# siravan/fib_tf

Hardware: AMD Instinct MI355X
Metric: million cell-steps/sec (grid_cells x timesteps / wall_s), 4v 512x512 (higher is better)
Workload: dtype f32; 1 GPU; fenton 512x512, dt=0.1 ms, phase-field hole, S1 + S2 pacing (BASELINE configs[1]); 1 step = 1 run() tick = 10 sub-steps; sub_steps_per_tick=10, fused_sub_steps_per_launch=10, launches_per_tick=1, ticks_per_launch=32, tile=44x25 cells, 3 rows per wave (chosen by measurement on the first tick), arithmetic=fast_math (default policy), parallelism=single device, setup_ticks=6001, timing=one region of 2647 ticks

## Files before the change

fib_tf_amd/_lib.py:

```python
import ctypes as C
import os
import subprocess

import numpy as np

HERE = os.path.dirname(os.path.abspath(__file__))
ROOT = os.path.dirname(HERE)
SO = os.path.join(HERE, 'libfibhip.so')
SRC = os.path.join(HERE, 'csrc', 'fibhip.hip')
HDR = os.path.join(ROOT, 'include', 'fibhip.h')

FENTON4V, BR, COURT, COURT_US, CUSTOM = 0, 1, 2, 3, 4
OBS_MAPS = ('first_up', 'last_up', 'prev_up', 'apd', 'count')
CHEBY, SKIP, CHRONIC, FAST, ALLVARS, ROW_INTERLEAVED, ZEROPAD, HOLD = 1, 2, 4, 8, 16, 32, 64, 128

HIPCC_FLAGS = ['-O3', '--offload-arch=gfx950', '-ffp-contract=off', '-fno-slp-vectorize', '-fvisibility=hidden', '-fPIC', '-shared',
               '-std=c++17', '-Wall', '-Wno-unused-value', '-Wno-unused-result']


def _build_tag(so_path):
    import re
    return '-DFIB_BUILD_TAG=b_' + re.sub(r'[^0-9A-Za-z_]', '_', os.path.splitext(os.path.basename(so_path))[0])


# ... 102 lines not shown
    'fibhip_comm_open': ([C.c_char_p], C.c_int),
    'fibhip_comm_unique_id': ([C.c_char_p], C.c_int),
    'fibhip_comm_check': ([_h, C.c_int, C.c_int], C.c_int),
    'fibhip_comm_init': ([_h, C.c_char_p, C.c_int, C.c_int], C.c_int),
    'fibhip_comm_exchange': ([_h, C.c_int, C.c_int], C.c_int),
    'fibhip_comm_free': ([_h], C.c_int),
    'fibhip_copy_bandwidth': ([C.c_int, C.c_size_t, C.c_int, _fp], C.c_int),
    'fibhip_warm': ([C.c_int], C.c_int),
    'fibhip_module_load': ([C.c_int, C.c_void_p, C.c_size_t, C.POINTER(ModuleDesc), C.POINTER(C.c_void_p)], C.c_int),
    'fibhip_module_unload': ([C.c_void_p], C.c_int),
    'fibhip_launch_plan': ([_h, _ip, _ip], C.c_int),
    'fibhip_get_state_direct': ([_h, C.c_int, _fp], C.c_int),
    'fibhip_host_alloc': ([C.c_size_t, C.POINTER(C.c_void_p)], C.c_int),
    'fibhip_host_free': ([C.c_void_p], C.c_int),
    'fibhip_ticks_per_launch': ([_h], C.c_int),
    'fibhip_launch_stats': ([_h, C.POINTER(C.c_longlong)], C.c_int),
    'fibhip_spec_stats': ([_h, C.POINTER(C.c_longlong)], C.c_int),
    'fibhip_fallbacks': ([_h, C.POINTER(C.c_longlong)], C.c_int),
    'fibhip_set_mt_wait_ms': ([_h, C.c_int], C.c_int),
    'fibhip_expect': ([_h, C.c_int], C.c_int),
    'fibhip_trace_begin': ([_h], C.c_int),
    'fibhip_trace_end': ([_h, C.POINTER(TraceEvent), C.c_int], C.c_int),
    'fibhip_plan_tile': ([_h, _ip, _ip, _ip], C.c_int),
    'fibhip_observe_begin': ([_h, C.c_int, C.c_float, C.c_float], C.c_int),
    'fibhip_observe_get': ([_h, C.c_int, C.c_void_p], C.c_int),
    'fibhip_observe_ticks': ([_h, C.POINTER(C.c_longlong)], C.c_int),
    'fibhip_observe_end': ([_h], C.c_int),
    'fibhip_electrode_begin': ([_h, C.c_int, C.c_int, _ip, _fp, C.c_int, C.c_longlong], C.c_int),
    'fibhip_electrode_count': ([_h, C.POINTER(C.c_longlong)], C.c_int),
    'fibhip_electrode_read': ([_h, C.c_longlong, C.c_longlong, _fp], C.c_int),
    'fibhip_electrode_end': ([_h], C.c_int),
    'fibhip_last_error': ([], C.c_char_p),
}

_lib = None


DEPS = [SRC, HDR] + [os.path.join(HERE, "csrc", f) for f in ("kernels.hpp", "models.hpp", "fenton_step.inc", "br_step.inc",
                                                             "court_step.inc", "court_inter.inc")]


def build(force=False, verbose=False):
    if not force and os.path.exists(SO) and all(os.path.getmtime(SO) >= os.path.getmtime(d) for d in DEPS):
        return SO
    hipcc = os.environ.get('HIPCC', '/opt/rocm/bin/hipcc')
    cmd = [hipcc] + HIPCC_FLAGS + [SRC, '-o', SO]
# ... 474 lines not shown
```

fib_tf_amd/csrc/fibhip.hip:

```cpp
#include <hip/hip_runtime.h>

#include <atomic>
#include <chrono>
#include <climits>
#include <cmath>
#include <cstdarg>
#include <cstdio>
#include <cstdlib>
#include <cstring>
#include <dlfcn.h>
#include <limits>
#include <mutex>
#include <new>
#include <vector>

#include "../../include/fibhip.h"
#include "kernels.hpp"

using namespace fib;

static thread_local char g_err[512] = "";

static int fail(int code, const char *fmt, ...)
{
// ... 61 lines not shown
}

template <class M, class P, int MODE, int K, int TX, int TY, int R, bool PHASE>
static hipError_t launch_strip(hipStream_t st, const LaunchCtx &c)
{
    Geo g = c.g;
    g.tiles_x = (g.W + TX - 1) / TX;
    g.ty_a = (g.r1 > g.r0) ? (g.r1 - g.r0 + TY - 1) / TY : 0;
    const int tiles_y = g.ty_a + ((g.rb1 > g.rb0) ? (g.rb1 - g.rb0 + TY - 1) / TY : 0);
    g.ntiles = g.tiles_x * tiles_y;
    if (g.ntiles <= 0) return hipSuccess;
    PtrTab<M::NVAR> pt;
    for (int v = 0; v < M::NVAR; ++v) {
        pt.in[v] = c.in[v];
        pt.out[v] = c.out[v];
    }
    constexpr int NT = 64 * ((TY + 2 * (K - 1) + R - 1) / R);
    const int grid = ((g.ntiles + 7) / 8) * 8;
    hipLaunchKernelGGL((strip_kernel<M, P, MODE, K, TX, TY, R, PHASE>), dim3(grid), dim3(NT), 0, st, g, pt, c.ph,
                       *static_cast<const typename M::Consts *>(c.consts), c.sub0);
    return hipGetLastError();
}

template <class M, class P, int MODE, int K, int TX, int TY, int R, bool PHASE>
static hipError_t launch_strip_mt(hipStream_t st, const LaunchCtx &c)
{
    Geo g = c.g;
    g.tiles_x = (g.W + TX - 1) / TX;
    g.ty_a = (g.r1 > g.r0) ? (g.r1 - g.r0 + TY - 1) / TY : 0;
    g.ntiles = g.tiles_x * g.ty_a;
    if (g.ntiles <= 0) return hipSuccess;
    PtrTab<M::NVAR> pt;
    for (int v = 0; v < M::NVAR; ++v) {
        pt.in[v] = c.in[v];
        pt.out[v] = c.out[v];
    }
    constexpr int NT = 64 * ((TY + 2 * (K - 1) + R - 1) / R);
    const int grid = ((g.ntiles + 7) / 8) * 8;
    hipLaunchKernelGGL((strip_mt_kernel<M, P, MODE, K, TX, TY, R, PHASE>), dim3(grid), dim3(NT), 0, st, g, pt, c.ph,
                       *static_cast<const typename M::Consts *>(c.consts), c.sub0, c.mt);
    return hipGetLastError();
}

template <class M, class P, int MODE, int K, int TX, int TY, int R, bool PHASE>
static hipError_t launch_rows(hipStream_t st, const LaunchCtx &c)
{
    Geo g = c.g;
    g.tiles_x = (g.W + TX - 1) / TX;
    g.ty_a = (g.r1 > g.r0) ? (g.r1 - g.r0 + TY - 1) / TY : 0;
    const int tiles_y = g.ty_a + ((g.rb1 > g.rb0) ? (g.rb1 - g.rb0 + TY - 1) / TY : 0);
    g.ntiles = g.tiles_x * tiles_y;
    if (g.ntiles <= 0) return hipSuccess;
    PtrTab<M::NVAR> pt;
    for (int v = 0; v < M::NVAR; ++v) {
        pt.in[v] = c.in[v];
        pt.out[v] = c.out[v];
    }
    constexpr int NT = 64 * ((TY + 2 * (K - 1) + R - 1) / R);
    const int grid = ((g.ntiles + 7) / 8) * 8;
    hipLaunchKernelGGL((rows_kernel<M, P, MODE, K, TX, TY, R, PHASE>), dim3(grid), dim3(NT), 0, st, g, pt, c.ph,
                       *static_cast<const typename M::Consts *>(c.consts), c.sub0);
    return hipGetLastError();
// ... 40 lines not shown
    auto put = [&](const void *p, size_t n, size_t align) {
        off = (off + align - 1) & ~(align - 1);
        memcpy(buf + off, p, n);
        off += n;
    };
    put(&g, sizeof g, alignof(Geo));
    off = (off + 7) & ~(size_t)7;
    memcpy(buf + off, c.in, (size_t)c.nvar * sizeof(void *));
    off += (size_t)c.nvar * sizeof(void *);
    memcpy(buf + off, c.out, (size_t)c.nvar * sizeof(void *));
    off += (size_t)c.nvar * sizeof(void *);
    if (c.kind != MK_POINTWISE) put(&c.ph, sizeof c.ph, alignof(PhaseTab));
    const char zeros[64] = {0};
    if (c.consts_bytes > 0) put(c.consts ? c.consts : zeros, (size_t)c.consts_bytes, 4);
    if (c.kind != MK_POINTWISE) put(&c.sub0, sizeof c.sub0, alignof(int));
    if (c.kind == MK_STRIP_MT) put(&c.mt, sizeof c.mt, alignof(MtArgs));
    void *config[] = {HIP_LAUNCH_PARAM_BUFFER_POINTER, buf, HIP_LAUNCH_PARAM_BUFFER_SIZE, &off, HIP_LAUNCH_PARAM_END};
    return hipModuleLaunchKernel(c.kern, grid, 1, 1, threads, 1, 1, 0, st, nullptr, config);
}

constexpr int VM_FENTON_ZP = 100;
constexpr int VM_COURT_AGG = 101;

struct Variant {
    int model, mode, fast, phase;
    int K, TX, TY, NT;
    launch_fn fn;
    hipFunction_t kern = nullptr;
    int kind = 0;
    launch_fn fn_mt = nullptr;
    hipFunction_t kern_mt = nullptr;
};

#define V4(MODEL, MID, MODE, K, TX, TY, NT)                                                        \
    {MID, MODE, 0, 0, K, TX, TY, NT, launch_tick<MODEL, Exact, MODE, K, TX, TY, NT, false>},       \
    {MID, MODE, 0, 1, K, TX, TY, NT, launch_tick<MODEL, Exact, MODE, K, TX, TY, NT, true>},        \
    {MID, MODE, 1, 0, K, TX, TY, NT, launch_tick<MODEL, Fast, MODE, K, TX, TY, NT, false>},        \
    {MID, MODE, 1, 1, K, TX, TY, NT, launch_tick<MODEL, Fast, MODE, K, TX, TY, NT, true>}

#define F2(MODEL, MID, MODE, K, TX, TY, NT)                                                        \
    {MID, MODE, 1, 0, K, TX, TY, NT, launch_tick<MODEL, Fast, MODE, K, TX, TY, NT, false>},        \
    {MID, MODE, 1, 1, K, TX, TY, NT, launch_tick<MODEL, Fast, MODE, K, TX, TY, NT, true>}

#define FS2(MODEL, MID, MODE, K, TX, TY, R)                                                        \
    {MID, MODE, 1, 0, K, TX, TY, -(R), launch_strip<MODEL, Fast, MODE, K, TX, TY, R, false>},      \
    {MID, MODE, 1, 1, K, TX, TY, -(R), launch_strip<MODEL, Fast, MODE, K, TX, TY, R, true>}

#define S4(MODEL, MID, MODE, K, TX, TY, R)                                                         \
    {MID, MODE, 0, 0, K, TX, TY, -(R), launch_strip<MODEL, Exact, MODE, K, TX, TY, R, false>},     \
    {MID, MODE, 0, 1, K, TX, TY, -(R), launch_strip<MODEL, Exact, MODE, K, TX, TY, R, true>},      \
    {MID, MODE, 1, 0, K, TX, TY, -(R), launch_strip<MODEL, Fast, MODE, K, TX, TY, R, false>},      \
    {MID, MODE, 1, 1, K, TX, TY, -(R), launch_strip<MODEL, Fast, MODE, K, TX, TY, R, true>}

#define S4M(MODEL, MID, MODE, K, TX, TY, R)                                                        \
    {MID, MODE, 0, 0, K, TX, TY, -(R), launch_strip<MODEL, Exact, MODE, K, TX, TY, R, false>, nullptr, 0,  \
     launch_strip_mt<MODEL, Exact, MODE, K, TX, TY, R, false>},                                    \
    {MID, MODE, 0, 1, K, TX, TY, -(R), launch_strip<MODEL, Exact, MODE, K, TX, TY, R, true>, nullptr, 0,   \
     launch_strip_mt<MODEL, Exact, MODE, K, TX, TY, R, true>},                                     \
    {MID, MODE, 1, 0, K, TX, TY, -(R), launch_strip<MODEL, Fast, MODE, K, TX, TY, R, false>, nullptr, 0,   \
     launch_strip_mt<MODEL, Fast, MODE, K, TX, TY, R, false>},                                     \
    {MID, MODE, 1, 1, K, TX, TY, -(R), launch_strip<MODEL, Fast, MODE, K, TX, TY, R, true>, nullptr, 0,    \
     launch_strip_mt<MODEL, Fast, MODE, K, TX, TY, R, true>}

#define W4(MODEL, MID, MODE, K, TX, TY, R)                                                         \
    {MID, MODE, 0, 0, K, TX, TY, -(32 + (R)), launch_rows<MODEL, Exact, MODE, K, TX, TY, R, false>},  \
    {MID, MODE, 0, 1, K, TX, TY, -(32 + (R)), launch_rows<MODEL, Exact, MODE, K, TX, TY, R, true>},   \
    {MID, MODE, 1, 0, K, TX, TY, -(32 + (R)), launch_rows<MODEL, Fast, MODE, K, TX, TY, R, false>},   \
    {MID, MODE, 1, 1, K, TX, TY, -(32 + (R)), launch_rows<MODEL, Fast, MODE, K, TX, TY, R, true>}

static const Variant g_variants[] = {
#ifdef FIB_CUSTOM_MODEL_INC
    V4(Custom, FIBHIP_CUSTOM, 0, 1, 64, 4, 256),
#if FIB_CUSTOM_K > 1
    S4(Custom, FIBHIP_CUSTOM, 0, FIB_CUSTOM_K, FIB_CUSTOM_TX, FIB_CUSTOM_TY, FIB_CUSTOM_R),
#if FIB_CUSTOM_TYB > 0
    S4(Custom, FIBHIP_CUSTOM, 0, FIB_CUSTOM_K, FIB_CUSTOM_TX, FIB_CUSTOM_TYB, FIB_CUSTOM_R),
#endif
#endif
#if FIB_CUSTOM_K2 > 1 && FIB_CUSTOM_K2 != FIB_CUSTOM_K
    S4(Custom, FIBHIP_CUSTOM, 0, FIB_CUSTOM_K2, FIB_CUSTOM_TX2, FIB_CUSTOM_TY2, FIB_CUSTOM_R2),
#endif
#endif
#ifndef FIB_CUSTOM_ONLY
#ifndef FIB_ONLY_BR
    S4M(Fenton, FIBHIP_FENTON4V, 0, 10, 44, 25, 3),
    S4M(Fenton, FIBHIP_FENTON4V, 0, 10, 44, 28, 3),
    S4M(Fenton, FIBHIP_FENTON4V, 0, 10, 44, 27, 3),
    S4M(Fenton, FIBHIP_FENTON4V, 0, 10, 44, 30, 3),
    S4M(Fenton, FIBHIP_FENTON4V, 0, 10, 44, 32, 4),
    S4M(Fenton, FIBHIP_FENTON4V, 0, 10, 44, 36, 4),
    S4M(Fenton, FIBHIP_FENTON4V, 0, 10, 44, 40, 4),
    S4M(Fenton, FIBHIP_FENTON4V, 0, 10, 44, 44, 4),
    S4(Fenton, FIBHIP_FENTON4V, 0, 5, 54, 21, 3),
    S4(Fenton, FIBHIP_FENTON4V, 0, 5, 54, 23, 3),
    S4(Fenton, FIBHIP_FENTON4V, 0, 5, 54, 22, 4),
    S4(Fenton, FIBHIP_FENTON4V, 0, 5, 54, 27, 3),
    S4(Fenton, FIBHIP_FENTON4V, 0, 5, 54, 25, 3),
    S4(Fenton, FIBHIP_FENTON4V, 0, 5, 54, 28, 3),
    S4(Fenton, FIBHIP_FENTON4V, 0, 5, 54, 31, 3),
    S4(Fenton, FIBHIP_FENTON4V, 0, 5, 54, 34, 3),
    S4(Fenton, FIBHIP_FENTON4V, 0, 5, 54, 32, 4),
    S4(Fenton, FIBHIP_FENTON4V, 0, 5, 54, 40, 3),
    S4(Fenton, FIBHIP_FENTON4V, 0, 5, 54, 44, 4),
    S4(Fenton, FIBHIP_FENTON4V, 0, 5, 54, 56, 4),
    S4(Fenton, FIBHIP_FENTON4V, 0, 2, 60, 18, 4),
    W4(Fenton, FIBHIP_FENTON4V, 0, 10, 44, 25, 3),
    W4(Fenton, FIBHIP_FENTON4V, 0, 5, 54, 21, 3),
    V4(Fenton, FIBHIP_FENTON4V, 0, 10, 32, 32, 512),
// ... 107 lines not shown
    int cur[FIB_MAXVAR];
    int nxt[FIB_MAXVAR];
    bool has_consts;
    Fenton::Consts kf;
    BeelerReuter::Consts kb;
    Courtemanche::Consts kc;
#ifdef FIB_CUSTOM_MODEL_INC
    Custom::Consts ku;
#endif
    std::vector<PlanItem> plan;
    hipEvent_t ev_main, ev_int, ev_t0, ev_t1;
    int phase_of_tick;
    long launches, t_launches0;
    int own0, own1;
    bool whole_in_edges;
    int pending;
    int multi_max;
    std::vector<PlanItem> plan_multi[4];
    float *xbuf;
    unsigned *epochs;
    unsigned epoch_base;
    bool epochs_stale;
    int mt_max;
    int mt_cur;
    long long n_ticks, n_mt_launches, n_mt_ticks;
    long long n_spec_kept, n_spec_redone;
    int mt_run, mt_run_prev;
    int spec_n, spec_used;
    int spec_nxt[FIB_MAXVAR];
    int mt_run_prev2;
    int hist[8], nhist;
    bool series_fresh;
    bool ahead_ok;
    unsigned spec_id;
    unsigned *host_word;
    unsigned *done_word, *done_word_dev;
    unsigned done_seq;
    bool no_stream_write;
    unsigned *snap_flags_dev;
    unsigned mt_ids;
    unsigned mt_seq;
    bool spec_trust;
    hipEvent_t ev_spec;
    unsigned *snap_flags;
    unsigned snap_seq;
    bool mt_inflight;
// ... 423 lines not shown
        const char *e = getenv("FIBHIP_AHEAD");
        h->ahead_ok = !(e && atoi(e) == 0) && h->own_slab;
    }
    h->n_fallbacks = h->n_replayed = 0;
    h->recovering = false;
    h->expect = 0;
    h->expect_fresh = false;
    h->ptr_exposed = false;
    {
        const char *e = getenv("FIBHIP_MT_WAIT_MS");
        h->mt_wait_ms = (e && atol(e) > 0) ? (unsigned)(atol(e) > 0xFFFFFFl ? 0xFFFFFFl : atol(e)) : 0u;
        const char *f = getenv("FIBHIP_MT_FAKE_GIVEUP");
        h->fake_giveup_at = (f && atol(f) > 0) ? atol(f) : 0;
        h->fake_seen = 0;
    }
    HIPCHK(hipEventCreateWithFlags(&h->ev_spec, hipEventDisableTiming));
    h->n_ticks = h->n_mt_launches = h->n_mt_ticks = h->n_spec_kept = h->n_spec_redone = 0;
    h->mt_inflight = false;
    h->dead = false;
    {
        hipDeviceProp_t prop;
        HIPCHK(hipGetDeviceProperties(&prop, desc->device));
        h->ncu = prop.multiProcessorCount;
        const char *e = getenv("FIBHIP_MT"), *em = getenv("FIBHIP_MT_MAX");
        h->mt_max = (e && atoi(e) == 0) ? 1 : (em && atoi(em) > 0 ? imin(atoi(em), 4096) : MT_MAX_TICKS);
        if (interleaved || desc->ghost_top || desc->ghost_bottom || (long long)h->cells * ((nv + 3) / 4 * 4) * 8 >= (1LL << 31))
            h->mt_max = 1;
        for (const char *var : {"HSA_CU_MASK", "ROC_GLOBAL_CU_MASK"}) {
            const char *m = getenv(var);
            if (m && *m) h->mt_max = 1;
        }
    }
    h->agg = nullptr;
    h->use_agg = false;
    h->agg_dirty = true;
    h->agg_ghost_dirty = false;
    h->agg_stride = 0;
#if !defined(FIB_CUSTOM_ONLY) && !defined(FIB_ONLY_BR)
    {
        const char *e = getenv("FIBHIP_COURT_AGG");
        const bool shard = desc->ghost_top || desc->ghost_bottom;
        if (desc->model == FIBHIP_COURT && (desc->flags & FIBHIP_FAST) && !(desc->flags & FIBHIP_ALLVARS) &&
            (h->own_slab || shard) && !(e && atoi(e) == 0)) {
            const bool il = h->pitch != desc->width;
            const size_t floats = il ? (size_t)desc->height * h->pitch : (size_t)CourtAgg::NAGG * h->cells;
            HIPCHK(hipMalloc((void **)&h->agg, floats * sizeof(float)));
// ... 625 lines not shown
    const bool trial = !commit && !nxt_out;
    if (!trial) {
        fibhip_ctx::MtRec rec;
        rec.id = h->mt_seq;
        rec.T = T;
        rec.counted = commit;
        memcpy(rec.src, h->cur, sizeof rec.src);
        h->journal.push_back(rec);
        if (h->fake_giveup_at > 0 && ++h->fake_seen == h->fake_giveup_at) {
            unsigned *w = (unsigned *)(h->probe_host + 12);
            *w = h->mt_seq;
            HIPCHK(hipMemcpyAsync(c.mt.err, w, sizeof(unsigned), hipMemcpyHostToDevice, h->s0));
            __atomic_store_n(h->host_word + MT_GIVEUP_WORD, h->mt_seq, __ATOMIC_RELEASE);
        }
    }
    {
        std::lock_guard<std::mutex> lock(g_mt.mu);
        fibhip_ctx *&owner = g_mt.owner[h->d.device];
        if (owner && owner != h) {
            HIPCHK(hipEventRecord(owner->ev_main, owner->s0));
            HIPCHK(hipStreamWaitEvent(h->s0, owner->ev_main, 0));
        }
        if (int rc = trace_open(h, h->s0, "strip_mt_kernel", v->K, v->TX, v->TY, v->NT, T)) return rc;
        HIPCHK(v->fn_mt(h->s0, c));
        if (int rc = trace_close(h, h->s0)) return rc;
        owner = h;
    }
    h->launches++;
    if (commit) {
        h->n_mt_launches++;
        h->n_mt_ticks += T;
        h->n_ticks += T;
    }
    h->mt_inflight = true;
    h->epoch_base += (unsigned)(T - 1);
    if (commit) memcpy(h->cur, nxt, sizeof nxt);
    if (nxt_out) memcpy(nxt_out, nxt, sizeof nxt);
    if (commit && h->el) return electrode_advance(h, T);
    return 0;
}

static int journal_bound(fibhip_ctx *h)
{
    if (h->journal.size() < 256 || h->spec_n > 0) return 0;
    return sync_s0(h);
}

// ... 1088 lines not shown
{
    if (!h) return fail(FIBHIP_EINVAL, "null handle");
    return ((h->d.ghost_top || h->d.ghost_bottom) && (h->cpos + h->pending) % h->cycle == h->cycle - 1) ? 1 : 0;
}

extern "C" int fibhip_plan_tile(fibhip_t h, int *tile_w, int *tile_h, int *rows_per_wave)
{
    if (!h) return fail(FIBHIP_EINVAL, "null handle");
    if (h->plan.empty()) return fail(FIBHIP_EINVAL, "no plan");
    const PlanItem &it = (h->multi_max > 1 && !h->plan_multi[h->multi_max].empty()) ? h->plan_multi[h->multi_max][0] : h->plan[0];
    if (tile_w) *tile_w = it.TX;
    if (tile_h) *tile_h = it.TY;
    if (rows_per_wave) *rows_per_wave = it.v ? -it.v->NT : 0;
    return 0;
}

extern "C" int fibhip_ticks_per_launch(fibhip_t h)
{
    if (!h) return fail(FIBHIP_EINVAL, "null handle");
    if (mt_variant(h)) return h->mt_max;
    return multi_cap(h);
}

extern "C" int fibhip_trace_begin(fibhip_t h)
{
    NEED(h);
    FLUSH(h);
    if (h->phase_of_tick) return fail(FIBHIP_EINVAL, "trace_begin inside an open tick");
    for (auto &r : h->trace) {
        if (r.e0) hipEventDestroy(r.e0);
        if (r.e1) hipEventDestroy(r.e1);
    }
    h->trace.clear();
    h->tracing = true;
    return 0;
}

extern "C" int fibhip_trace_end(fibhip_t h, fibhip_trace_event *out, int max_events)
{
    NEED(h);
    if (!h->tracing) return fail(FIBHIP_EINVAL, "trace_end without trace_begin");
    if (!out || max_events < 1) return fail(FIBHIP_EINVAL, "trace_end: bad argument");
    FLUSH(h);
    h->tracing = false;
    HIPCHK(wait_stream(h->s1));
    SYNC_S0(h);
// ... 244 lines not shown
```

fib_tf_amd/csrc/kernels.hpp:

```cpp
#pragma once
#include "models.hpp"

namespace fib {
FIB_TAG_BEGIN

struct Geo {
    int H, W;
    int pitch;
    int Hg;
    int row_off;
    int r0, r1;
    int rb0, rb1;
    int ty_a;
    int tiles_x, ntiles;
};

static FIB_DEV void tile_rows(const Geo &g, int by, int TY, int &y0, int &rend)
{
    if (by < g.ty_a) {
        y0 = g.r0 + by * TY;
        rend = g.r1;
    } else {
        y0 = g.rb0 + (by - g.ty_a) * TY;
        rend = g.rb1;
// ... 351 lines not shown
    static constexpr bool value = false;
};
template <class M>
struct HasPinnedSpare<M, void_of<decltype(&M::pinned_spare)>> {
    static constexpr bool value = true;
};
template <class A, class B>
struct SameType {
    static constexpr bool value = false;
};
template <class A>
struct SameType<A, A> {
    static constexpr bool value = true;
};
template <class M, bool SPARE, class C>
static FIB_DEV decltype(auto) pinned_for(const C &k)
{
    if constexpr (SPARE && HasPinnedSpare<M>::value)
        return M::pinned_spare(k);
    else
        return M::pinned(k);
}

template <class M, class P, int MODE, int K, int TX, int TY, int R, bool PHASE, bool MT>
static FIB_DEV void strip_body(const Geo &g, const PtrTab<M::NVAR> &pt, const PhaseTab &ph, const typename M::Consts &k, int sub0,
                               const MtArgs &mt)
{
    constexpr int NV = M::NVAR;
    constexpr int CX = TX + 2 * (K - 1), CY = TY + 2 * (K - 1);
    static_assert(CX <= 62 && K > 1, "strip_kernel: compute box must fit 62 lanes");
    static_assert(!MT || (CX == 62 && TX >= K && TY >= K), "multi-tick launches: 62-column box, the rim inside the eight neighbours");
    constexpr int NW = (CY + R - 1) / R;
    constexpr int LP = 64, LQ = NW * R + 2, NL = LP * LQ;
    constexpr unsigned WMASK = M::mask(MODE);
    constexpr bool PAIR = MT && (R % 2 == 0);
    constexpr int SPARE = PAIR ? R + 6 : R + 4;
    __shared__ __attribute__((aligned(16))) float lds[2][NL + SPARE * 64];
    __shared__ int mt_abort;
    __shared__ float snapl[MT ? NW * R * 64 : 1];

    const int tile = xcd_tile(blockIdx.x, g.ntiles);
    if (tile >= g.ntiles) return;
    FIB_STAMP(0);
    if (MT && threadIdx.x == 0) mt_abort = 0;
    auto &&kk = pinned_for<M, (MT && SameType<P, Exact>::value)>(k);
    const int lane = threadIdx.x & 63;
    const int wave = __builtin_amdgcn_readfirstlane(threadIdx.x >> 6);
    const int by = tile / g.tiles_x, bx = tile - by * g.tiles_x;
    int y0, rend;
    tile_rows(g, by, TY, y0, rend);
    const int x0 = bx * TX;
    const int cx0 = x0 - (K - 1), cy0 = y0 - (K - 1);
    const int gx = cx0 - 1 + lane;
    const int c0 = wave * R;

    const int bW = clampi(gx - 1, 1, g.W - 2), bC = clampi(gx, 1, g.W - 2), bE = clampi(gx + 1, 1, g.W - 2);
    const int jW = clampi(bW - (cx0 - 1), 0, 63), jC = clampi(bC - (cx0 - 1), 0, 63), jE = clampi(bE - (cx0 - 1), 0, 63);
    auto brow = [&](int grow) {
        return clampi(clampi(grow, 1, g.Hg - 2) - g.row_off, 0, g.H - 1);
    };

    const float *vin = pt.in[0];
    float win[R + 2][3];
#pragma unroll
    for (int q = 0; q < R + 2; ++q) {
        const float *row = vin + (size_t)brow(cy0 + c0 - 1 + q + g.row_off) * g.pitch;
        win[q][0] = row[bW];
        win[q][1] = row[bC];
        win[q][2] = row[bE];
    }
    const bool lane_in = lane >= 1 && lane <= CX && gx >= 0 && gx < g.W;
    const bool col_border = gx == 0 || gx == g.W - 1;
    const bool store_col = lane_in && gx >= x0 && gx < x0 + TX;
    const bool wr = lane_in && !col_border;
    float s[R][NV];
    PhaseCoef<P> pc[R];
    int off[R];
    bool own[R];
#pragma unroll
    for (int r = 0; r < R; ++r) {
        const int gy = cy0 + c0 + r;
        const int oy = clampi(gy, 0, g.H - 1), ox = clampi(gx, 0, g.W - 1);
        off[r] = oy * g.pitch + ox;
        own[r] = store_col && gy >= y0 && gy < min(y0 + TY, rend) && gy < g.H;
#pragma unroll
        for (int v = 0; v < NV; ++v) s[r][v] = pt.in[v][off[r]];
        if (PHASE) pc[r].load(ph, oy * g.W + ox);
    }
    const int snap_at = (MT && mt.snap) ? ((int)(mt.ticks_id & 0xFFFFu) >= 3 ? 1 : 0) : -1;
    if constexpr (MT) {
        if (mt.snap) {
#pragma unroll
            for (int r = 0; r < R; ++r) {
                float x = s[r][0];
#pragma unroll
                for (int v = 1; v < NV; ++v) x = (mt.snap_var & 0xFF) == v ? s[r][v] : x;
                snapl[(c0 + r) * 64 + lane] = x;
            }
        }
    }
    const bool top_open = cy0 + g.row_off > 0, bot_open = cy0 + CY + g.row_off < g.Hg;
    const int aW = PAIR ? (c0 >> 1) * 128 + 2 * jW : c0 * LP + jW, aC = PAIR ? (c0 >> 1) * 128 + 2 * jC : c0 * LP + jC,
              aE = PAIR ? (c0 >> 1) * 128 + 2 * jE : c0 * LP + jE;
    auto ro = [](int k) constexpr { return PAIR ? ((1 + k) >> 1) * 128 + ((1 + k) & 1) : k * LP; };
    auto cell_at = [](int row, int col) { return PAIR ? (row >> 1) * 128 + 2 * col : row * LP + col; };
    constexpr int SPARE_ROW = PAIR ? LQ + 3 : LQ + 2;
    auto window = [&](const float *Bq, float (&w)[R + 2][3]) {
        if constexpr (PAIR) {
            typedef float v2f __attribute__((ext_vector_type(2)));
#pragma unroll
            for (int m = 0; m < (R + 2) / 2; ++m) {
                int oW = aW + m * 128, oC = aC + m * 128, oE = aE + m * 128;
                if (m > 0) asm volatile("" : "+v"(oW));
                const v2f a = *reinterpret_cast<const v2f *>(Bq + oW);
                if (m > 0) asm volatile("" : "+v"(oC));
                const v2f b = *reinterpret_cast<const v2f *>(Bq + oC);
                if (m > 0) asm volatile("" : "+v"(oE));
                const v2f c = *reinterpret_cast<const v2f *>(Bq + oE);
                w[2 * m][0] = a.x; w[2 * m + 1][0] = a.y;
                w[2 * m][1] = b.x; w[2 * m + 1][1] = b.y;
                w[2 * m][2] = c.x; w[2 * m + 1][2] = c.y;
            }
        } else {
#pragma unroll
            for (int q = 0; q < R + 2; ++q) {
                w[q][0] = Bq[aW + q * LP];
                w[q][1] = Bq[aC + q * LP];
                w[q][2] = Bq[aE + q * LP];
            }
        }
    };
    const int g0 = cy0 + c0 + g.row_off;
    const int ra_fix = max(max(0, -g0), -(cy0 + c0));
    const int rb_fix = min(min(R, CY - c0), min(g.Hg - g.row_off, g.H) - (cy0 + c0));
    unsigned pub = 0;
    int top_r = -1, bot_r = -1;
#pragma unroll
    for (int r = 0; r < R; ++r) {
        if (g0 + r != 0 && g0 + r != g.Hg - 1) pub |= 1u << r;
        if (g0 + r == 1) top_r = r;
        if (g0 + r == g.Hg - 2) bot_r = r;
    }
    const int wi = wr ? cell_at(c0 + 1, lane) : cell_at(SPARE_ROW, lane);
    FIB_STAMP(1);
    __builtin_amdgcn_s_waitcnt(0x0F70);
    FIB_STAMP(2);

    constexpr int STEP_UNROLL = 2;
    constexpr int WHOLE_NVR = 12;
    constexpr bool WHOLE_LOOP = MT && NV * R <= WHOLE_NVR;
    const bool whole = WHOLE_LOOP && ra_fix == 0 && rb_fix == R && (!top_open || c0 >= K - 1) && (!bot_open || c0 + R <= CY - (K - 1)) &&
                       pub == (1u << R) - 1u && top_r < 0 && bot_r < 0;
#pragma unroll 1
    for (int tick = 0;; ++tick) {
    unsigned hw = 0u;
    if constexpr (MT) {
        if (tile == 0 && threadIdx.x == 0) {
            typedef const __attribute__((address_space(1))) unsigned *gptr;
            gptr p = (gptr)(mt.snap_flag + MT_HOST_WORD_AT);
            asm volatile("" : "+s"(p));
            hw = __hip_atomic_load(p, __ATOMIC_RELAXED, __HIP_MEMORY_SCOPE_SYSTEM);
        }
    }
    if constexpr (MT) {
        if (tick == snap_at) {
#pragma unroll
            for (int r = 0; r < R; ++r)
                if (own[r]) __hip_atomic_store(mt.snap + off[r], snapl[(c0 + r) * 64 + lane], __ATOMIC_RELAXED, __HIP_MEMORY_SCOPE_SYSTEM);
        }
    }
    if (WHOLE_LOOP && whole) {
#pragma unroll STEP_UNROLL
        for (int st = 0; st < K; ++st) {
            float *B = lds[(st & 1) ^ 1];
            float lp[R], cc[R];
#pragma unroll
            for (int r = 0; r < R; ++r) {
                float l = lap9<P>(win[r][1], win[r + 2][1], win[r + 1][0], win[r + 1][2], win[r][0], win[r + 2][0],
                                  win[r][2], win[r + 2][2], win[r + 1][1]);
                if (PHASE) l = pc[r].add(l, win[r][1], win[r + 2][1], win[r + 1][0], win[r + 1][2]);
                lp[r] = l;
                cc[r] = win[r + 1][1];
            }
            if constexpr (M::HAS_VEC) {
                M::template stepN<P, MODE, R>(s, cc, lp, kk, sub0 + st);
            } else {
#pragma unroll
                for (int r = 0; r < R; ++r) M::template step<P, MODE>(s[r], cc[r], lp[r], kk, sub0 + st);
            }
            if (st + 1 < K) {
#pragma unroll
// ... 133 lines not shown
                    }
                    break;
                }
                __builtin_amdgcn_s_sleep(MT_POLL_SLEEP);
            }
        }
        FIB_BSTAMP(4);
        __syncthreads();
        FIB_BSTAMP(5);
        if (mt_abort == 1) {
            if (threadIdx.x == 0) {
                const unsigned who = __hip_atomic_load(mt.err, __ATOMIC_RELAXED, __HIP_MEMORY_SCOPE_AGENT);
                if (who != 0u)
                    __hip_atomic_store(mt.snap_flag + MT_HOST_WORD_AT + MT_GIVEUP_WORD, who, __ATOMIC_RELAXED, __HIP_MEMORY_SCOPE_SYSTEM);
            }
            return;
        }
        if (mt_abort == 2) {
            if (threadIdx.x == 0) __hip_atomic_fetch_add(mt.err + 2 * MT_EPOCH_STRIDE, 1u, __ATOMIC_RELAXED, __HIP_MEMORY_SCOPE_AGENT);
            break;
        }
#pragma unroll
        for (int r = 0; r < R; ++r) {
            if (!own[r]) {
#pragma unroll
                for (int c = 0; c < NC4; ++c) {
                    const fib_v4f v = __builtin_bit_cast(
                        fib_v4f, __builtin_amdgcn_raw_buffer_load_b128(rs, (int)(pbase + c * plane16 + (unsigned)off[r] * 16u), 0, 16));
                    s[r][4 * c] = v.x;
                    if (4 * c + 1 < NV) s[r][4 * c + 1 < NV ? 4 * c + 1 : 0] = v.y;
                    if (4 * c + 2 < NV) s[r][4 * c + 2 < NV ? 4 * c + 2 : 0] = v.z;
                    if (4 * c + 3 < NV) s[r][4 * c + 3 < NV ? 4 * c + 3 : 0] = v.w;
                }
            }
        }
        const int gtop = cy0 - 1 + g.row_off, gbot = cy0 + CY + g.row_off;
        const int cxx = clampi(gx, 0, g.W - 1);
        float ring = 0.0f;
        const bool ring_top = wave == 0 && gtop >= 1 && gtop <= g.Hg - 2;
        const bool ring_bot = wave == NW - 1 && gbot >= 1 && gbot <= g.Hg - 2;
        if (ring_top)
            ring = __builtin_bit_cast(float, __builtin_amdgcn_raw_buffer_load_b32(rs, (int)(pbase + (unsigned)((cy0 - 1) * g.W + cxx) * 16u), 0, 16));
        if (ring_bot)
            ring = __builtin_bit_cast(float, __builtin_amdgcn_raw_buffer_load_b32(rs, (int)(pbase + (unsigned)((cy0 + CY) * g.W + cxx) * 16u), 0, 16));
        FIB_BSTAMP_WAIT();
        FIB_BSTAMP(6);
        float *B0 = lds[0];
        const int wib = (gx >= 1 && gx <= g.W - 2) ? cell_at(c0 + 1, lane) : cell_at(SPARE_ROW, lane);
        {
            const unsigned live = ra_fix < rb_fix ? ((1u << rb_fix) - 1u) & ~((1u << ra_fix) - 1u) : 0u;
            const unsigned m = live & pub;
#pragma unroll
            for (int r = 0; r < R; ++r)
                if ((m >> r) & 1u) B0[wib + ro(r)] = s[r][0];
            if (top_r >= 0 || bot_r >= 0) {
#pragma unroll
                for (int r = 0; r < R; ++r) {
                    if (r == top_r && ((live >> r) & 1u)) {
                        B0[wib + ro(r - 1)] = s[r][0];
                        if (c0 + r >= 1) B0[wib + ro(r - 2)] = s[r][0];
                    }
                    if (r == bot_r && ((live >> r) & 1u)) {
                        B0[wib + ro(r + 1)] = s[r][0];
// ... 13 lines not shown
        FIB_BSTAMP_WAIT();
        FIB_BSTAMP(9);
    }
    }

#pragma unroll
    for (int r = 0; r < R; ++r) {
        if (own[r]) {
#pragma unroll
            for (int v = 0; v < NV; ++v)
                if ((WMASK >> v) & 1u) pt.out[v][off[r]] = s[r][v];
        }
    }
    FIB_STAMP(14);
}

template <class M, class P, int MODE, int K, int TX, int TY, int R, bool PHASE>
__global__ void __launch_bounds__(64 * ((TY + 2 * (K - 1) + R - 1) / R))
strip_kernel(Geo g, PtrTab<M::NVAR> pt, PhaseTab ph, typename M::Consts k, int sub0)
{
    strip_body<M, P, MODE, K, TX, TY, R, PHASE, false>(g, pt, ph, k, sub0, MtArgs{});
}

template <class M, class P, int MODE, int K, int TX, int TY, int R, bool PHASE>
__global__ void __launch_bounds__(64 * ((TY + 2 * (K - 1) + R - 1) / R))
strip_mt_kernel(Geo g, PtrTab<M::NVAR> pt, PhaseTab ph, typename M::Consts k, int sub0, MtArgs mt)
{
    g.pitch = g.W;
    g.Hg = g.H;
    g.row_off = 0;
    g.r0 = 0;
    g.r1 = g.H;
    g.rb0 = g.rb1 = 0;
    g.ty_a = 0x7fffffff;
    strip_body<M, P, MODE, K, TX, TY, R, PHASE, true>(g, pt, ph, k, sub0, mt);
}

static FIB_DEV float lane_west(float v)
{
    return __builtin_bit_cast(float, __builtin_amdgcn_update_dpp(0, __builtin_bit_cast(int, v), 0x138, 0xF, 0xF, true));
}
static FIB_DEV float lane_east(float v)
{
    return __builtin_bit_cast(float, __builtin_amdgcn_update_dpp(0, __builtin_bit_cast(int, v), 0x130, 0xF, 0xF, true));
}
static FIB_DEV float lane_get(float v, int lane)
{
    return __builtin_bit_cast(float, __builtin_amdgcn_readlane(__builtin_bit_cast(int, v), lane));
}

template <class P, bool PHASE>
static FIB_DEV float stencil9_lanes(float N, float S, float C, const PhaseCoef<P> &pc)
{
    const float ns = N + S;
    const float Wv = lane_west(C), E = lane_east(C);
    const float l1 = (ns + Wv) + E, d = (lane_west(ns) + lane_east(N)) + lane_east(S);
    float r;
    if constexpr (same_type<P, Fast>::value)
// ... 397 lines not shown
```

include/fibhip.h:

```cpp
#ifndef FIBHIP_H
#define FIBHIP_H

#ifdef __cplusplus
extern "C" {
#endif
#if defined(__GNUC__) || defined(__clang__)
#pragma GCC visibility push(default)
#endif

#define FIBHIP_ABI_VERSION 1

typedef struct fibhip_ctx *fibhip_t;

enum fibhip_model {
    FIBHIP_FENTON4V = 0, FIBHIP_BR = 1, FIBHIP_COURT = 2,
    FIBHIP_COURT_US = 3,
    FIBHIP_CUSTOM = 4
};

enum fibhip_flags {
    FIBHIP_CHEBY   = 1u << 0,
    FIBHIP_SKIP    = 1u << 1,
    FIBHIP_CHRONIC = 1u << 2,
    FIBHIP_FAST    = 1u << 3,
// ... 99 lines not shown
    int struct_size;
    int nvar;
    int steps_per_tick;
    int nmodes;
    unsigned masks[8];
    int consts_bytes;
    int K, TX, TY, R, TYB, K2, TX2, TY2, R2;
    int nkernels;
    const fibhip_module_kernel *kernels;
} fibhip_module_desc;
typedef struct fibhip_module *fibhip_module_t;
int fibhip_module_load(int device, const void *code, size_t nbytes, const fibhip_module_desc *d, fibhip_module_t *out);
int fibhip_module_unload(fibhip_module_t m);

int fibhip_copy_bandwidth(int device, size_t nbytes, int reps, float *gb_per_s);

int fibhip_warm(int device);

#define FIBHIP_COURT_NINTER 32
int fibhip_court_inter(int device, int n, const float *V, int fast, float *out);

int fibhip_launch_plan(fibhip_t h, int *fused_steps, int *launches_per_tick);
int fibhip_plan_tile(fibhip_t h, int *tile_w, int *tile_h, int *rows_per_wave);
int fibhip_ticks_per_launch(fibhip_t h);
int fibhip_launch_stats(fibhip_t h, long long out[4]);
int fibhip_spec_stats(fibhip_t h, long long out[2]);
int fibhip_fallbacks(fibhip_t h, long long out[2]);
int fibhip_set_mt_wait_ms(fibhip_t h, int ms);

typedef struct fibhip_trace_event {
    char name[96];
    double start_us, dur_us;
    int K, tile_w, tile_h, rows_per_wave, ticks;
} fibhip_trace_event;
int fibhip_trace_begin(fibhip_t h);
int fibhip_trace_end(fibhip_t h, fibhip_trace_event *out, int max_events);

enum fibhip_obs_map { FIBHIP_OBS_FIRST_UP = 0, FIBHIP_OBS_LAST_UP = 1, FIBHIP_OBS_PREV_UP = 2, FIBHIP_OBS_APD = 3, FIBHIP_OBS_COUNT = 4 };
int fibhip_observe_begin(fibhip_t h, int var, float up, float down);
int fibhip_observe_get(fibhip_t h, int which, void *dst);
int fibhip_observe_ticks(fibhip_t h, long long *k);
int fibhip_observe_end(fibhip_t h);

#define FIBHIP_MAX_ELECTRODES 64
int fibhip_electrode_begin(fibhip_t h, int var, int n, const int *rects, const float *weights, int every, long long capacity);
int fibhip_electrode_count(fibhip_t h, long long *samples);
// ... 13 lines not shown
```

Measured before the change: 226,700 Mcell-steps/s.

## Add table-driven row-strip layouts for multi-tick strip kernel waves

Adds compile-time tables that assign arbitrary row strips to waves in the multi-tick strip kernel, with a validity check that every row is covered exactly once. For the 44x25, K=10, R=3 Fenton tile, the Fast variants now default to layout 2, which uses 16 waves with a reordered strip assignment and a split last strip instead of 15 contiguous waves. An environment variable can override the choice. The aim is to rebalance the waves, which adds one wave per workgroup and table lookups for strip offsets.

```diff
diff --git a/fib_tf_amd/_lib.py b/fib_tf_amd/_lib.py
--- a/fib_tf_amd/_lib.py
+++ b/fib_tf_amd/_lib.py
@@ -148,6 +148,7 @@
     'fibhip_trace_begin': ([_h], C.c_int),
     'fibhip_trace_end': ([_h, C.POINTER(TraceEvent), C.c_int], C.c_int),
     'fibhip_plan_tile': ([_h, _ip, _ip, _ip], C.c_int),
+    'fibhip_strip_layout': ([C.c_int, C.c_int, C.c_int, C.c_int, _ip, _ip], C.c_int),
     'fibhip_observe_begin': ([_h, C.c_int, C.c_float, C.c_float], C.c_int),
     'fibhip_observe_get': ([_h, C.c_int, C.c_void_p], C.c_int),
     'fibhip_observe_ticks': ([_h, C.POINTER(C.c_longlong)], C.c_int),
diff --git a/fib_tf_amd/csrc/fibhip.hip b/fib_tf_amd/csrc/fibhip.hip
--- a/fib_tf_amd/csrc/fibhip.hip
+++ b/fib_tf_amd/csrc/fibhip.hip
@@ -107,7 +107,7 @@
     return hipGetLastError();
 }
 
-template <class M, class P, int MODE, int K, int TX, int TY, int R, bool PHASE>
+template <class M, class P, int MODE, int K, int TX, int TY, int R, bool PHASE, int LAYOUT = 0>
 static hipError_t launch_strip_mt(hipStream_t st, const LaunchCtx &c)
 {
     Geo g = c.g;
@@ -120,9 +120,10 @@
         pt.in[v] = c.in[v];
         pt.out[v] = c.out[v];
     }
-    constexpr int NT = 64 * ((TY + 2 * (K - 1) + R - 1) / R);
+    constexpr int NT = 64 * StripLayout<K, TY, R, LAYOUT>::NW;
+    static_assert(NT <= 1024, "a workgroup has at most 1024 threads");
     const int grid = ((g.ntiles + 7) / 8) * 8;
-    hipLaunchKernelGGL((strip_mt_kernel<M, P, MODE, K, TX, TY, R, PHASE>), dim3(grid), dim3(NT), 0, st, g, pt, c.ph,
+    hipLaunchKernelGGL((strip_mt_kernel<M, P, MODE, K, TX, TY, R, PHASE, LAYOUT>), dim3(grid), dim3(NT), 0, st, g, pt, c.ph,
                        *static_cast<const typename M::Consts *>(c.consts), c.sub0, c.mt);
     return hipGetLastError();
 }
@@ -209,6 +210,7 @@
 constexpr int VM_FENTON_ZP = 100;
 constexpr int VM_COURT_AGG = 101;
 
+constexpr int MT_LAYOUTS = 3;
 struct Variant {
     int model, mode, fast, phase;
     int K, TX, TY, NT;
@@ -217,6 +219,8 @@
     int kind = 0;
     launch_fn fn_mt = nullptr;
     hipFunction_t kern_mt = nullptr;
+    launch_fn fn_mt_lay[MT_LAYOUTS + 1] = {nullptr};
+    int lay_default = 0;
 };
 
 #define V4(MODEL, MID, MODE, K, TX, TY, NT)                                                        \
@@ -248,6 +252,17 @@
      launch_strip_mt<MODEL, Fast, MODE, K, TX, TY, R, false>},                                     \
     {MID, MODE, 1, 1, K, TX, TY, -(R), launch_strip<MODEL, Fast, MODE, K, TX, TY, R, true>, nullptr, 0,    \
      launch_strip_mt<MODEL, Fast, MODE, K, TX, TY, R, true>}
+
+#define S4ML_ONE(MODEL, MID, MODE, K, TX, TY, R, POL, FAST, PH, LDEF)                                                            \
+    {MID, MODE, FAST, PH, K, TX, TY, -(R), launch_strip<MODEL, POL, MODE, K, TX, TY, R, PH>, nullptr, 0,                       \
+     launch_strip_mt<MODEL, POL, MODE, K, TX, TY, R, PH>, nullptr,                                                              \
+     {nullptr, launch_strip_mt<MODEL, POL, MODE, K, TX, TY, R, PH, 1>, launch_strip_mt<MODEL, POL, MODE, K, TX, TY, R, PH, 2>, \
+      launch_strip_mt<MODEL, POL, MODE, K, TX, TY, R, PH, 3>}, LDEF}
+#define S4ML(MODEL, MID, MODE, K, TX, TY, R, LF, LE)                                               \
+    S4ML_ONE(MODEL, MID, MODE, K, TX, TY, R, Exact, 0, false, LE),                                 \
+    S4ML_ONE(MODEL, MID, MODE, K, TX, TY, R, Exact, 0, true, LE),                                  \
+    S4ML_ONE(MODEL, MID, MODE, K, TX, TY, R, Fast, 1, false, LF),                                  \
+    S4ML_ONE(MODEL, MID, MODE, K, TX, TY, R, Fast, 1, true, LF)
 
 #define W4(MODEL, MID, MODE, K, TX, TY, R)                                                         \
     {MID, MODE, 0, 0, K, TX, TY, -(32 + (R)), launch_rows<MODEL, Exact, MODE, K, TX, TY, R, false>},  \
@@ -270,7 +285,7 @@
 #endif
 #ifndef FIB_CUSTOM_ONLY
 #ifndef FIB_ONLY_BR
-    S4M(Fenton, FIBHIP_FENTON4V, 0, 10, 44, 25, 3),
+    S4ML(Fenton, FIBHIP_FENTON4V, 0, 10, 44, 25, 3, 2, 0),
     S4M(Fenton, FIBHIP_FENTON4V, 0, 10, 44, 28, 3),
     S4M(Fenton, FIBHIP_FENTON4V, 0, 10, 44, 27, 3),
     S4M(Fenton, FIBHIP_FENTON4V, 0, 10, 44, 30, 3),
@@ -424,6 +439,7 @@
     unsigned epoch_base;
     bool epochs_stale;
     int mt_max;
+    int strip_layout;
     int mt_cur;
     long long n_ticks, n_mt_launches, n_mt_ticks;
     long long n_spec_kept, n_spec_redone;
@@ -893,6 +909,8 @@
         hipDeviceProp_t prop;
         HIPCHK(hipGetDeviceProperties(&prop, desc->device));
         h->ncu = prop.multiProcessorCount;
+        const char *el = getenv("FIBHIP_STRIP_LAYOUT");
+        h->strip_layout = (el && *el) ? imin(atoi(el) < 0 ? -1 : atoi(el), MT_LAYOUTS) : -1;
         const char *e = getenv("FIBHIP_MT"), *em = getenv("FIBHIP_MT_MAX");
         h->mt_max = (e && atoi(e) == 0) ? 1 : (em && atoi(em) > 0 ? imin(atoi(em), 4096) : MT_MAX_TICKS);
         if (interleaved || desc->ghost_top || desc->ghost_bottom || (long long)h->cells * ((nv + 3) / 4 * 4) * 8 >= (1LL << 31))
@@ -1564,7 +1582,8 @@
             HIPCHK(hipStreamWaitEvent(h->s0, owner->ev_main, 0));
         }
         if (int rc = trace_open(h, h->s0, "strip_mt_kernel", v->K, v->TX, v->TY, v->NT, T)) return rc;
-        HIPCHK(v->fn_mt(h->s0, c));
+        const int lay = h->strip_layout >= 0 ? h->strip_layout : v->lay_default;
+        HIPCHK((lay > 0 && lay <= MT_LAYOUTS && v->fn_mt_lay[lay] ? v->fn_mt_lay[lay] : v->fn_mt)(h->s0, c));
         if (int rc = trace_close(h, h->s0)) return rc;
         owner = h;
     }
@@ -2699,6 +2718,37 @@
     return multi_cap(h);
 }
 
+template <int K, int TY, int R, int LAYOUT>
+static int strip_layout_out(int *c0, int *rows)
+{
+    typedef StripLayout<K, TY, R, LAYOUT> SL;
+    for (int w = 0; w < SL::NW; ++w) {
+        c0[w] = SL::host_c0(w);
+        rows[w] = SL::host_rows(w);
+    }
+    return SL::NW;
+}
+
+extern "C" int fibhip_strip_layout(int K, int tile_h, int rows_per_wave, int layout, int *c0, int *rows)
+{
+    if (!c0 || !rows || K < 2 || tile_h < 1 || rows_per_wave < 1) return fail(FIBHIP_EINVAL, "strip_layout: bad argument");
+    const int CY = tile_h + 2 * (K - 1), R = rows_per_wave, NW = (CY + R - 1) / R;
+    if (layout == 0) {
+        if (NW > 16) return fail(FIBHIP_EINVAL, "strip_layout: more than 16 waves");
+        for (int w = 0; w < NW; ++w) {
+            c0[w] = w * R;
+            rows[w] = imin(R, CY - w * R);
+        }
+        return NW;
+    }
+    if (K == 10 && tile_h == 25 && R == 3) {
+        if (layout == 1) return strip_layout_out<10, 25, 3, 1>(c0, rows);
+        if (layout == 2) return strip_layout_out<10, 25, 3, 2>(c0, rows);
+        if (layout == 3) return strip_layout_out<10, 25, 3, 3>(c0, rows);
+    }
+    return fail(FIBHIP_EINVAL, "strip_layout: no such table for this tile shape");
+}
+
 extern "C" int fibhip_trace_begin(fibhip_t h)
 {
     NEED(h);
diff --git a/fib_tf_amd/csrc/kernels.hpp b/fib_tf_amd/csrc/kernels.hpp
--- a/fib_tf_amd/csrc/kernels.hpp
+++ b/fib_tf_amd/csrc/kernels.hpp
@@ -397,7 +397,72 @@
         return M::pinned(k);
 }
 
-template <class M, class P, int MODE, int K, int TX, int TY, int R, bool PHASE, bool MT>
+template <int NWAVES>
+struct StripTable {
+    int c0[NWAVES], rows[NWAVES];
+};
+template <int K, int TY, int R, int LAYOUT>
+struct StripLayout {
+    static_assert(LAYOUT == 0, "no such strip layout for this tile shape");
+    static constexpr int CY = TY + 2 * (K - 1);
+    static constexpr int NW = (CY + R - 1) / R;
+    static constexpr int LQ = NW * R + 2;
+    static FIB_DEV int c0(int wave) { return wave * R; }
+    static FIB_DEV int rows(int) { return R; }
+    static FIB_DEV bool first(int wave) { return wave == 0; }
+    static FIB_DEV bool last(int wave) { return wave == NW - 1; }
+    static constexpr int host_c0(int wave) { return wave * R; }
+    static constexpr int host_rows(int wave) { return CY - wave * R < R ? CY - wave * R : R; }
+};
+template <int K, int TY, int R, int NWAVES>
+struct StripLayoutTable {
+    static constexpr int CY = TY + 2 * (K - 1);
+    static constexpr int NW = NWAVES;
+    static_assert(NW <= 16, "a workgroup has at most 16 waves");
+    static constexpr unsigned long long pack(const int *v, int from, int bits)
+    {
+        unsigned long long x = 0;
+        for (int i = 0; i < 64 / bits && from + i < NW; ++i) x |= (unsigned long long)v[from + i] << (i * bits);
+        return x;
+    }
+    static constexpr int max_c0(const int *v)
+    {
+        int m = 0;
+        for (int i = 0; i < NW; ++i) m = v[i] > m ? v[i] : m;
+        return m;
+    }
+    static constexpr bool valid(const StripTable<NW> &t)
+    {
+        int seen[CY] = {};
+        for (int w = 0; w < NW; ++w) {
+            if (t.rows[w] < 1 || t.rows[w] > R || t.c0[w] < 0 || t.c0[w] + t.rows[w] > CY) return false;
+            for (int r = 0; r < t.rows[w]; ++r) seen[t.c0[w] + r]++;
+        }
+        for (int y = 0; y < CY; ++y)
+            if (seen[y] != 1) return false;
+        return true;
+    }
+};
+#define FIB_STRIP_LAYOUT(K_, TY_, R_, LAYOUT_, NWAVES_, ...)                                                                    \
+    template <>                                                                                                                  \
+    struct StripLayout<K_, TY_, R_, LAYOUT_> : StripLayoutTable<K_, TY_, R_, NWAVES_> {                                          \
+        typedef StripLayoutTable<K_, TY_, R_, NWAVES_> B;                                                                        \
+        static constexpr StripTable<NWAVES_> T = __VA_ARGS__;                                                                    \
+        static_assert(B::valid(T), "strip layout: rows not covered exactly once, or a strip too high");                          \
+        static constexpr int LQ = B::max_c0(T.c0) + R_ + 2;           \
+        static constexpr unsigned long long C_LO = B::pack(T.c0, 0, 8), C_HI = B::pack(T.c0, 8, 8), ROWS = B::pack(T.rows, 0, 4); \
+        static FIB_DEV int c0(int wave) { return (int)(((wave < 8 ? C_LO : C_HI) >> ((wave & 7) * 8)) & 0xFFull); }              \
+        static FIB_DEV int rows(int wave) { return (int)((ROWS >> (wave * 4)) & 0xFull); }                                       \
+        static FIB_DEV bool first(int wave) { return c0(wave) == 0; }                                                            \
+        static FIB_DEV bool last(int wave) { return c0(wave) + rows(wave) == B::CY; }                                            \
+        static constexpr int host_c0(int wave) { return T.c0[wave]; }                                                            \
+        static constexpr int host_rows(int wave) { return T.rows[wave]; }                                                        \
+    }
+FIB_STRIP_LAYOUT(10, 25, 3, 1, 15, {{0, 33, 6, 9, 12, 15, 18, 21, 24, 27, 30, 3, 34, 37, 40}, {3, 1, 3, 3, 3, 3, 3, 3, 3, 3, 3, 3, 3, 3, 3}});
+FIB_STRIP_LAYOUT(10, 25, 3, 2, 16, {{0, 33, 6, 9, 12, 15, 18, 21, 24, 27, 30, 3, 34, 37, 40, 42}, {3, 1, 3, 3, 3, 3, 3, 3, 3, 3, 3, 3, 3, 3, 2, 1}});
+FIB_STRIP_LAYOUT(10, 25, 3, 3, 15, {{0, 9, 6, 3, 12, 15, 18, 21, 24, 27, 28, 31, 34, 37, 40}, {3, 3, 3, 3, 3, 3, 3, 3, 3, 1, 3, 3, 3, 3, 3}});
+
+template <class M, class P, int MODE, int K, int TX, int TY, int R, bool PHASE, bool MT, int LAYOUT = 0>
 static FIB_DEV void strip_body(const Geo &g, const PtrTab<M::NVAR> &pt, const PhaseTab &ph, const typename M::Consts &k, int sub0,
                                const MtArgs &mt)
 {
@@ -405,10 +470,13 @@
     constexpr int CX = TX + 2 * (K - 1), CY = TY + 2 * (K - 1);
     static_assert(CX <= 62 && K > 1, "strip_kernel: compute box must fit 62 lanes");
     static_assert(!MT || (CX == 62 && TX >= K && TY >= K), "multi-tick launches: 62-column box, the rim inside the eight neighbours");
-    constexpr int NW = (CY + R - 1) / R;
-    constexpr int LP = 64, LQ = NW * R + 2, NL = LP * LQ;
+    typedef StripLayout<K, TY, R, LAYOUT> SL;
+    static_assert(LAYOUT == 0 || MT, "strip layouts by table: multi-tick launches only");
+    constexpr int NW = SL::NW;
+    constexpr int LP = 64, LQ = SL::LQ, NL = LP * LQ;
     constexpr unsigned WMASK = M::mask(MODE);
     constexpr bool PAIR = MT && (R % 2 == 0);
+    static_assert(!PAIR || LAYOUT == 0, "the paired image needs every strip to start on an even row");
     constexpr int SPARE = PAIR ? R + 6 : R + 4;
     __shared__ __attribute__((aligned(16))) float lds[2][NL + SPARE * 64];
     __shared__ int mt_abort;
@@ -427,7 +495,7 @@
     const int x0 = bx * TX;
     const int cx0 = x0 - (K - 1), cy0 = y0 - (K - 1);
     const int gx = cx0 - 1 + lane;
-    const int c0 = wave * R;
+    const int c0 = SL::c0(wave);
 
     const int bW = clampi(gx - 1, 1, g.W - 2), bC = clampi(gx, 1, g.W - 2), bE = clampi(gx + 1, 1, g.W - 2);
     const int jW = clampi(bW - (cx0 - 1), 0, 63), jC = clampi(bC - (cx0 - 1), 0, 63), jE = clampi(bE - (cx0 - 1), 0, 63);
@@ -457,7 +525,7 @@
         const int gy = cy0 + c0 + r;
         const int oy = clampi(gy, 0, g.H - 1), ox = clampi(gx, 0, g.W - 1);
         off[r] = oy * g.pitch + ox;
-        own[r] = store_col && gy >= y0 && gy < min(y0 + TY, rend) && gy < g.H;
+        own[r] = store_col && gy >= y0 && gy < min(y0 + TY, rend) && gy < g.H && (LAYOUT == 0 || r < SL::rows(wave));
 #pragma unroll
         for (int v = 0; v < NV; ++v) s[r][v] = pt.in[v][off[r]];
         if (PHASE) pc[r].load(ph, oy * g.W + ox);
@@ -470,7 +538,7 @@
                 float x = s[r][0];
 #pragma unroll
                 for (int v = 1; v < NV; ++v) x = (mt.snap_var & 0xFF) == v ? s[r][v] : x;
-                snapl[(c0 + r) * 64 + lane] = x;
+                snapl[(wave * R + r) * 64 + lane] = x;
             }
         }
     }
@@ -507,7 +575,7 @@
     };
     const int g0 = cy0 + c0 + g.row_off;
     const int ra_fix = max(max(0, -g0), -(cy0 + c0));
-    const int rb_fix = min(min(R, CY - c0), min(g.Hg - g.row_off, g.H) - (cy0 + c0));
+    const int rb_fix = min(min(SL::rows(wave), CY - c0), min(g.Hg - g.row_off, g.H) - (cy0 + c0));
     unsigned pub = 0;
     int top_r = -1, bot_r = -1;
 #pragma unroll
@@ -541,7 +609,7 @@
         if (tick == snap_at) {
 #pragma unroll
             for (int r = 0; r < R; ++r)
-                if (own[r]) __hip_atomic_store(mt.snap + off[r], snapl[(c0 + r) * 64 + lane], __ATOMIC_RELAXED, __HIP_MEMORY_SCOPE_SYSTEM);
+                if (own[r]) __hip_atomic_store(mt.snap + off[r], snapl[(wave * R + r) * 64 + lane], __ATOMIC_RELAXED, __HIP_MEMORY_SCOPE_SYSTEM);
         }
     }
     if (WHOLE_LOOP && whole) {
@@ -721,7 +789,7 @@
         }
 #pragma unroll
         for (int r = 0; r < R; ++r) {
-            if (!own[r]) {
+            if (!own[r] && (LAYOUT == 0 || r < rb_fix)) {
 #pragma unroll
                 for (int c = 0; c < NC4; ++c) {
                     const fib_v4f v = __builtin_bit_cast(
@@ -736,8 +804,8 @@
         const int gtop = cy0 - 1 + g.row_off, gbot = cy0 + CY + g.row_off;
         const int cxx = clampi(gx, 0, g.W - 1);
         float ring = 0.0f;
-        const bool ring_top = wave == 0 && gtop >= 1 && gtop <= g.Hg - 2;
-        const bool ring_bot = wave == NW - 1 && gbot >= 1 && gbot <= g.Hg - 2;
+        const bool ring_top = SL::first(wave) && gtop >= 1 && gtop <= g.Hg - 2;
+        const bool ring_bot = SL::last(wave) && gbot >= 1 && gbot <= g.Hg - 2;
         if (ring_top)
             ring = __builtin_bit_cast(float, __builtin_amdgcn_raw_buffer_load_b32(rs, (int)(pbase + (unsigned)((cy0 - 1) * g.W + cxx) * 16u), 0, 16));
         if (ring_bot)
@@ -797,8 +865,8 @@
     strip_body<M, P, MODE, K, TX, TY, R, PHASE, false>(g, pt, ph, k, sub0, MtArgs{});
 }
 
-template <class M, class P, int MODE, int K, int TX, int TY, int R, bool PHASE>
-__global__ void __launch_bounds__(64 * ((TY + 2 * (K - 1) + R - 1) / R))
+template <class M, class P, int MODE, int K, int TX, int TY, int R, bool PHASE, int LAYOUT = 0>
+__global__ void __launch_bounds__((64 * StripLayout<K, TY, R, LAYOUT>::NW))
 strip_mt_kernel(Geo g, PtrTab<M::NVAR> pt, PhaseTab ph, typename M::Consts k, int sub0, MtArgs mt)
 {
     g.pitch = g.W;
@@ -808,7 +876,7 @@
     g.r1 = g.H;
     g.rb0 = g.rb1 = 0;
     g.ty_a = 0x7fffffff;
-    strip_body<M, P, MODE, K, TX, TY, R, PHASE, true>(g, pt, ph, k, sub0, mt);
+    strip_body<M, P, MODE, K, TX, TY, R, PHASE, true, LAYOUT>(g, pt, ph, k, sub0, mt);
 }
 
 static FIB_DEV float lane_west(float v)
diff --git a/include/fibhip.h b/include/fibhip.h
--- a/include/fibhip.h
+++ b/include/fibhip.h
@@ -145,6 +145,7 @@
 
 int fibhip_launch_plan(fibhip_t h, int *fused_steps, int *launches_per_tick);
 int fibhip_plan_tile(fibhip_t h, int *tile_w, int *tile_h, int *rows_per_wave);
+int fibhip_strip_layout(int K, int tile_h, int rows_per_wave, int layout, int *c0, int *rows);
 int fibhip_ticks_per_launch(fibhip_t h);
 int fibhip_launch_stats(fibhip_t h, long long out[4]);
 int fibhip_spec_stats(fibhip_t h, long long out[2]);
```

Result: faster. 229,900 Mcell-steps/s, median of 6 (+1.4%).
